# i3drobotics/i3dr_stereo_camera-ros

Hardware: AMD Instinct MI355X
Metric: stereo pairs/sec + ms/frame, 1920×1080 D=256 8-path SGM, 1/2/4/8 MI355X (higher is better)
Workload: dtype u8

## Files before the change

### i3dr_stereo_camera-ros_amd/csrc/census_sgm.hip

```cpp
#include "sgm_device.h"
#include "sgm_launch.h"

#include <atomic>
#include <string>

#ifndef SGM_WPE
#define SGM_WPE 4
#endif
#ifndef SGM_WPE32
#define SGM_WPE32 4
#endif
#ifndef SGM_NT_STORE
#define SGM_NT_STORE 1
#endif
#ifndef SGM_NT_LOAD
#define SGM_NT_LOAD 1
#endif
#ifndef SGM_EXP
#define SGM_EXP 0
#endif
#if SGM_EXP != 0 && !defined(SGM_EXPERIMENT_BUILD)
#error "SGM_EXP builds give invalid results: define SGM_EXPERIMENT_BUILD as well (never in a release build)"
#endif
#ifndef SGM_LRPRIO_HW
#define SGM_LRPRIO_HW 37
#endif
#ifndef SGM_LRPRIO_DIAG
#define SGM_LRPRIO_DIAG 64
#endif
#ifndef SGM_UPWTA_PRIO
#define SGM_UPWTA_PRIO 0
#endif
#ifndef SGM_ROWS_LPL8
#define SGM_ROWS_LPL8 0
#endif
#ifndef SGM_P32
#define SGM_P32 1
#endif

#include <algorithm>
#include <cstdio>
#include <cstdlib>
#include <vector>

namespace sgm {

#define SGM_CENSUS_BIT(B)                                                              \
    asm("v_cmp_lt_u32_sdwa vcc, %1, %2 src0_sel:BYTE_" #B " src1_sel:DWORD\n\t"      \
        "v_addc_co_u32_e32 %0, vcc, %0, %0, vcc"                                       \
        : "+v"(acc) : "v"(w), "v"(c) : "vcc")
__device__ __forceinline__ void census_bit(uint32_t& acc, uint32_t w, uint32_t c, int b)
{
    switch (b) {
    case 0: SGM_CENSUS_BIT(0); break;
    case 1: SGM_CENSUS_BIT(1); break;
    case 2: SGM_CENSUS_BIT(2); break;
    default: SGM_CENSUS_BIT(3); break;
    }
}
#undef SGM_CENSUS_BIT

template <int PITCH>
__device__ __forceinline__ uint64_t census_code_lds(const uint8_t* tile, int ty, int tx)
{
    static_assert(PITCH % 4 == 0, "u32 rows");
    const uint32_t* t32 = (const uint32_t*)tile + (PITCH / 4) * ty + (tx >> 2);
    const int sb = tx & 3;
    const uint32_t c = tile[(ty + 3) * PITCH + tx + 4];
    uint32_t lo = 0, hi = 0;
#pragma unroll
    for (int dy = 6; dy >= 0; dy--) {
        const uint32_t* r = t32 + (PITCH / 4) * dy;
        const uint32_t w0 = r[0], w1 = r[1], w2 = r[2];
        const uint32_t a0 = __builtin_amdgcn_alignbyte(w1, w0, sb);
        const uint32_t a1 = __builtin_amdgcn_alignbyte(w2, w1, sb);
        const uint32_t a2 = __builtin_amdgcn_alignbyte(w2, w2, sb);
#pragma unroll
        for (int dx = 8; dx >= 0; dx--) {
            if (dy == 3 && dx == 4) continue;
            const int k = dy * 9 + dx - (dy * 9 + dx > 31 ? 1 : 0);
            const uint32_t w = dx < 4 ? a0 : dx < 8 ? a1 : a2;
            if (k >= 32) census_bit(hi, w, c, dx & 3);
            else census_bit(lo, w, c, dx & 3);
        }
    }
    return (uint64_t)lo | ((uint64_t)hi << 32);
}

__global__ __launch_bounds__(256) void k_census9x7(const uint8_t* __restrict__ L, const uint8_t* __restrict__ R,
                                                   size_t stride, int W, int H,
                                                   uint64_t* __restrict__ cL, uint64_t* __restrict__ cR, int ch, int gray)
{
    __shared__ __attribute__((aligned(16))) uint8_t tile[10 * 72];
    const uint8_t* img = blockIdx.z ? R : L;
    uint64_t* out = blockIdx.z ? cR : cL;
    const int x0 = blockIdx.x * 64, y0 = blockIdx.y * 4;
    if (ch == 3) {
        for (int i = threadIdx.x; i < 10 * 72; i += 256) {
            int ty = i / 72, tx = i - ty * 72;
            int yy = min(max(y0 + ty - 3, 0), H - 1), xx = min(max(x0 + tx - 4, 0), W - 1);
            const uint8_t* s = img + (size_t)yy * stride + 3 * xx;
            tile[i] = (uint8_t)gray_px(s[0], s[1], s[2], gray);
        }
    } else {
        for (int i = threadIdx.x; i < 10 * 72; i += 256) {
            int ty = i / 72, tx = i - ty * 72;
            int yy = min(max(y0 + ty - 3, 0), H - 1), xx = min(max(x0 + tx - 4, 0), W - 1);
            tile[i] = img[(size_t)yy * stride + xx];
        }
    }
    __syncthreads();
    const int tx = threadIdx.x & 63, ty = threadIdx.x >> 6;
    const int x = x0 + tx, y = y0 + ty;
    if (x >= W || y >= H) return;
    out[(size_t)y * W + x] = census_code_lds<72>(tile, ty, tx);
}

template <int DPL>
__device__ __forceinline__ void wload(const uint8_t* src, uint32_t (&wd)[(DPL + 3) / 4])
{
    if constexpr (DPL == 2) { wd[0] = *(const uint16_t*)src; }
    else if constexpr (DPL == 4) { wd[0] = *(const uint32_t*)src; }
    else if constexpr (DPL == 8) { const uint2 v = *(const uint2*)src; wd[0] = v.x; wd[1] = v.y; }
    else {
#pragma unroll
        for (int q = 0; q < DPL / 16; q++) {
            const uint4 v = ((const uint4*)src)[q];
            wd[4 * q] = v.x; wd[4 * q + 1] = v.y; wd[4 * q + 2] = v.z; wd[4 * q + 3] = v.w;
        }
    }
}

template <int DPL>
__device__ __forceinline__ void wload_buf(const uint8_t* base, uint32_t off, uint32_t (&wd)[(DPL + 3) / 4])
{
    const __amdgpu_buffer_rsrc_t rs = __builtin_amdgcn_make_buffer_rsrc((void*)base, 0, 0x7FFFFFFF, 0x00020000);
    constexpr int aux = SGM_NT_LOAD ? 2 : 0;
    if constexpr (DPL == 2) { wd[0] = __builtin_amdgcn_raw_buffer_load_b16(rs, off, 0, aux); }
    else if constexpr (DPL == 4) { wd[0] = __builtin_amdgcn_raw_buffer_load_b32(rs, off, 0, aux); }
    else if constexpr (DPL == 8) {
        const auto v = __builtin_amdgcn_raw_buffer_load_b64(rs, off, 0, aux);
        wd[0] = v[0]; wd[1] = v[1];
    } else {
#pragma unroll
        for (int q = 0; q < DPL / 16; q++) {
            const auto v = __builtin_amdgcn_raw_buffer_load_b128(rs, off + 16 * q, 0, aux);
            wd[4 * q] = v[0]; wd[4 * q + 1] = v[1]; wd[4 * q + 2] = v[2]; wd[4 * q + 3] = v[3];
        }
    }
}

template <int DPL>
__device__ __forceinline__ void store_pairs(uint8_t* dst, uint8_t* dst_hi, const uint32_t (&L)[DPL / 2])
{
    if constexpr (DPL == 2) {
        const uint16_t v = (uint16_t)__builtin_amdgcn_perm(0u, L[0], 0x0c0c0200u);
        if constexpr (SGM_NT_STORE) __builtin_nontemporal_store(v, (uint16_t*)dst);
        else *(uint16_t*)dst = v;
    } else if constexpr (DPL == 4) {
        const uint32_t v = __builtin_amdgcn_perm(L[1], L[0], 0x06040200u);
        if constexpr (SGM_NT_STORE) __builtin_nontemporal_store(v, (uint32_t*)dst);
        else *(uint32_t*)dst = v;
    } else if constexpr (DPL == 8) {
        typedef unsigned int v2u __attribute__((ext_vector_type(2)));
        const v2u v = {__builtin_amdgcn_perm(L[1], L[0], 0x06040200u), __builtin_amdgcn_perm(L[3], L[2], 0x06040200u)};
        if constexpr (SGM_NT_STORE) __builtin_nontemporal_store(v, (v2u*)dst);
        else *(v2u*)dst = v;
    } else {
        typedef unsigned int v4u __attribute__((ext_vector_type(4)));
#pragma unroll
        for (int q = 0; q < DPL / 16; q++) {
            const v4u v = {__builtin_amdgcn_perm(L[8 * q + 1], L[8 * q + 0], 0x06040200u),
                           __builtin_amdgcn_perm(L[8 * q + 3], L[8 * q + 2], 0x06040200u),
                           __builtin_amdgcn_perm(L[8 * q + 5], L[8 * q + 4], 0x06040200u),
                           __builtin_amdgcn_perm(L[8 * q + 7], L[8 * q + 6], 0x06040200u)};
            v4u* d = (v4u*)(q == 0 ? dst : dst_hi);
            if constexpr (SGM_NT_STORE) __builtin_nontemporal_store(v, d);
            else *d = v;
        }
    }
}

constexpr uint32_t kBaseP = 0x6400u, kBaseP2 = 0x64006400u;
constexpr uint32_t kInfP = 0x7000u, kInfP2 = 0x70007000u;
// ... 117 lines not shown
    HChunk16 c;
    c.cl = cLr[min(max(x, 0), g.W - 1)];
    const int xr = DX > 0 ? x + 1 - g.minD : x - g.minD - LPL * DPL;
    c.inj = cRr[min(max(xr, 0), g.W - 1)];
    return c;
}

template <int DPL, bool EXACT, int DX, bool PRIO = false, int LPL = 16>
__device__ __forceinline__ void p16_horiz(const uint64_t* __restrict__ cL, const uint64_t* __restrict__ cR,
                                          uint8_t* __restrict__ V, uint8_t* __restrict__ trash, const Geom& g,
                                          int y0)
{
    static_assert(LPL == 16 || LPL == 32, "horizontal scans: 16- or 32-lane lines");
    constexpr int M = DPL / 2;
    constexpr int U = DPL > 16 ? DPL : 16;
    const int lane = threadIdx.x & 63;
    const int r = lane / LPL, p = lane % LPL;
    const int y = y0 + r;
    const bool rowok = y < g.H;
    const int yc = min(y, g.H - 1);
    const uint64_t* cLr = cL + (size_t)yc * g.W;
    const uint64_t* cRr = cR + (size_t)yc * g.W;
    uint32_t imask[M], start[M];
    make_imask<DPL, EXACT, LPL>(p, g.D, imask, start);
    const uint32_t P1P1 = (uint32_t)g.P1 * 0x10001u, P2P2 = ((uint32_t)g.P2 + kBaseP) * 0x10001u;
    const int n = g.width1;
    const int xfirst = DX > 0 ? g.minX1 : g.maxX1 - 1;
    uint64_t cr[DPL];
#pragma unroll
    for (int k = 0; k < DPL; k++) cr[k] = cRr[min(max(xfirst - g.minD - p * DPL - k, 0), g.W - 1)];
    uint32_t Lr[M];
#pragma unroll
    for (int i = 0; i < M; i++) Lr[i] = start[i];
    uint8_t* rowbase = V + (size_t)yc * g.width1 * g.D + p * DPL;
    uint8_t* tr = trash + lane * DPL;
    const bool lane_ok = rowok && (EXACT || p * DPL < g.D);
    const bool hi_ok = EXACT || p * DPL + 16 < g.D;
    HChunk16 cur = hload16<DPL, DX, LPL>(cLr, cRr, g, 0, lane & 15);
    HChunk16 nxt = cur;
    for (int b = 0; b * U < n; b++) {
        if constexpr (PRIO) lr_prio(((n - b * U) * SGM_LRPRIO_HW) >> 6, g.H);
        static_for<0, U>([&](auto tc) {
            constexpr int t = decltype(tc)::value;
            if constexpr (t % 16 == 0) nxt = hload16<DPL, DX, LPL>(cLr, cRr, g, (b * U + t) / 16 + 1, lane & 15);
            const int i = b * U + t;
            const uint64_t cl = row_bcast_u64<t % 16>(cur.cl);
            const uint64_t inj = row_bcast_u64<t % 16>(cur.inj);
            uint32_t Labs[M];
            p16_step<DPL, EXACT, LPL>(Lr, cl, [&](int k) { return cr[DX > 0 ? ((k - t) % DPL + DPL) % DPL : (k + t) % DPL]; },
                                      P1P1, P2P2, imask, Labs);
            const int x1 = DX > 0 ? i : n - 1 - i;
            const bool ok = lane_ok && i < n;
            uint8_t* dst = ok ? rowbase + (size_t)x1 * g.D : tr;
            store_pairs<DPL>(dst, (ok && hi_ok) ? dst + 16 : tr + 16, Labs);
            if constexpr (DX > 0) {
                constexpr int ph = ((DPL - 1 - t) % DPL + DPL) % DPL;
                cr[ph] = LPL == 32 ? line32_shr1_u64(cr[ph], inj) : row_shr1_u64(cr[ph], inj);
            } else {
                constexpr int ph = t % DPL;
                cr[ph] = LPL == 32 ? line32_shl1_u64(cr[ph], inj) : row_shl1_u64(cr[ph], inj);
            }
            if constexpr (t % 16 == 15) cur = nxt;
        });
    }
}

template <int DPL, int LPL>
struct RowSeg {
    static constexpr int NL = kWG / LPL;
    static constexpr int NSEG = LPL * DPL + NL - 1;
    static constexpr int NPAD = LPL >= 16 ? NSEG + NSEG / 16 + 1 : NSEG + 4 * (NSEG / 32) + 4;
    static constexpr int NTOT = NSEG + NL;
    static constexpr int NLOAD = (NTOT + kWG - 1) / kWG;
    static constexpr int BUF = NPAD + NL + kWG;
    static __device__ __forceinline__ int phys(int e) { return LPL >= 16 ? e + (e >> 4) : e + 4 * (e >> 5); }
};
template <int DPL16>
struct RowsCfg {
#if SGM_ROWS_LPL8
    static constexpr int LPL = DPL16 <= 16 ? 8 : LineCfg<DPL16>::LPL;
#else
    static constexpr int LPL = LineCfg<DPL16>::LPL;
#endif
    static constexpr int DPL = DPL16 * 16 / LPL;
    static constexpr int NL = kWG / LPL;
};

template <int DPL, int LPL>
using SegRegs = uint64_t[RowSeg<DPL, LPL>::NLOAD];
template <int DPL, int LPL>
struct SegAddr {
    uint32_t off[RowSeg<DPL, LPL>::NLOAD];
    const char* lo;
};
template <int DPL, int LPL>
__device__ __forceinline__ SegAddr<DPL, LPL> seg_addr(const uint64_t* cL, const uint64_t* cR, const Geom& g, int tid)
{
    using RS = RowSeg<DPL, LPL>;
    SegAddr<DPL, LPL> a;
    const uint64_t* base = cL < cR ? cL : cR;
    const int bias = LPL * DPL + max(g.minD, 0);
    a.lo = (const char*)base - (size_t)8 * bias;
#pragma unroll
    for (int m = 0; m < RS::NLOAD; m++) {
        const int q = min(tid + m * kWG, RS::NTOT - 1);
        const int rel = q < RS::NSEG ? (int)(cR - base) + q - g.minD - LPL * DPL + 1 : (int)(cL - base) + (q - RS::NSEG);
        a.off[m] = (uint32_t)(8 * (rel + bias));
    }
    return a;
}
template <int DPL, int LPL>
__device__ __forceinline__ void seg_load(SegRegs<DPL, LPL>& v, const SegAddr<DPL, LPL>& a,
                                         const Geom& g, int rx, int ry, int xb, int s)
{
    const int y = ry > 0 ? s : g.H - 1 - s;
    const int yc = (SGM_EXP & 1) ? 0 : min(max(y, 0), g.H - 1);
    const char* sb = a.lo + (size_t)8 * ((size_t)yc * g.W + (xb + rx * s));
#pragma unroll
    for (int m = 0; m < RowSeg<DPL, LPL>::NLOAD; m++) v[m] = *(const uint64_t*)(sb + a.off[m]);
}

template <int DPL, int LPL>
__device__ __forceinline__ void seg_store(uint64_t* buf, const SegRegs<DPL, LPL>& v, int tid)
{
    using RS = RowSeg<DPL, LPL>;
#pragma unroll
    for (int m = 0; m < RS::NLOAD; m++) {
        const int q0 = tid + m * kWG;
        const int at = q0 < RS::NSEG ? RS::phys(q0) : (q0 < RS::NTOT ? RS::NPAD + (q0 - RS::NSEG) : RS::NPAD + RS::NL + tid);
        buf[at] = v[m];
    }
}

template <int DPL, bool EXACT, int LPL>
__device__ __forceinline__ void p16_seed(const uint8_t* src, const uint32_t (&imask)[DPL / 2], uint32_t (&Lr)[DPL / 2])
{
    uint32_t wd[(DPL + 3) / 4], Labs[DPL / 2];
    wload<DPL>(src, wd);
#pragma unroll
    for (int i = 0; i < DPL / 2; i++) {
        const uint32_t pr = __builtin_amdgcn_perm(0u, wd[i / 2], (i & 1) ? 0x0c030c02u : 0x0c010c00u);
        Labs[i] = pr | kBaseP2;
        if (!EXACT) Labs[i] = pk_max(Labs[i], imask[i]);
    }
    p16_relative<DPL, LPL>(Labs, Lr);
}

struct UpWta {
    const uint8_t* vols;
    size_t vol_bytes;
    uint64_t* res;
};
struct WtaPix { int best, minS, d16; bool rej; };
template <int DPL, bool EXACT>
__device__ __forceinline__ WtaPix wta_pix16(const uint32_t (&E)[(DPL + 3) / 4], const uint32_t (&O)[(DPL + 3) / 4],
                                            int p, const Geom& g, float inv_u, uint32_t* srow);
template <int DPL, bool EXACT>
__device__ __forceinline__ void wta_emask(int p, const Geom& g, uint32_t (&emaskE)[(DPL + 3) / 4],
                                          uint32_t (&emaskO)[(DPL + 3) / 4]);
template <int DPL>
__host__ __device__ constexpr size_t upwta_lds_bytes() { return (size_t)8 * 2 * RowSeg<DPL, 16>::BUF + (size_t)16 * 32 * ((DPL + 3) / 4) * 4; }

template <int DPL, bool EXACT, int LPL, bool FUSE = false, bool PRIO = false, int NP = 8>
__device__ __forceinline__ void p16_rows(const uint64_t* __restrict__ cL, const uint64_t* __restrict__ cR,
                                         uint8_t* __restrict__ V, uint8_t* __restrict__ trash, const Geom& g, int dir,
                                         int xb, const PathLaunch16& pl, uint64_t* lds, const UpWta& uw = UpWta{})
{
    static_assert(!FUSE || LPL == 16, "up+WTA blocks use 16 lanes per line (the WTA layout)");
    using RS = RowSeg<DPL, LPL>;
    constexpr int M = DPL / 2;
    constexpr int NL = RS::NL;
    const int tid = threadIdx.x;
    const int lane = tid & 63, w = tid >> 6;
    const int r = lane >> 4;
    const int p = LPL == 32 ? lane & 31 : LPL == 16 ? lane & 15 : (lane & 15) >> 1;
    const int j = LPL == 32 ? 2 * w + (lane >> 5) : LPL == 16 ? 4 * w + r : 8 * w + 2 * r + (lane & 1);
    const int rx = dir_rx(dir), ry = dir_ry(dir);
    int s0, s1;
    if (rx == 0) { s0 = 0; s1 = g.H; }
    else if (rx > 0) { s0 = max(0, g.minX1 - xb - (NL - 1)); s1 = min(g.H, g.maxX1 - xb); }
    else { s0 = max(0, xb - g.maxX1 + 1); s1 = min(g.H, xb + NL - g.minX1); }
    if (s0 >= s1) return;
    uint32_t imask[M], start[M];
    make_imask<DPL, EXACT, LPL>(p, g.D, imask, start);
    const uint32_t P1P1 = (uint32_t)g.P1 * 0x10001u, P2P2 = ((uint32_t)g.P2 + kBaseP) * 0x10001u;
    uint32_t Lr[M];
#pragma unroll
    for (int i = 0; i < M; i++) Lr[i] = start[i];
    bool pv = false;
    const uint8_t* bnd = pl.bnd[ry > 0 ? 0 : 1];
    if (bnd && s0 == 0) {
        const int x = xb + j, xp = x - rx;
        const bool cont = x >= g.minX1 && x < g.maxX1 && xp >= g.minX1 && xp < g.maxX1;
        const int xs = min(max(xp, g.minX1), g.maxX1 - 1) - g.minX1;
        uint32_t Ls[M];
        p16_seed<DPL, EXACT, LPL>(bnd + bnd_slot_of(dir) * pl.bnd_slot + (size_t)xs * g.D + p * DPL, imask, Ls);
#pragma unroll
        for (int i = 0; i < M; i++) Lr[i] = cont ? Ls[i] : Lr[i];
        pv = cont;
    }
    const bool lane_act = EXACT || p * DPL < g.D;
    const bool hi_ok = EXACT || p * DPL + 16 < g.D;
    uint8_t* const tr = trash + (tid & 63) * DPL;
    const int e_hi = j + (LPL - p) * DPL - 1;

    uint64_t* buf0 = lds;
    uint64_t* buf1 = lds + RS::BUF;
    uint64_t R0[RS::NLOAD], R1[RS::NLOAD], R2[RS::NLOAD], R3[RS::NLOAD];
    const SegAddr<DPL, LPL> sa = seg_addr<DPL, LPL>(cL, cR, g, tid);
    seg_load<DPL, LPL>(R0, sa, g, rx, ry, xb, s0);
    seg_store<DPL, LPL>(buf0, R0, tid);
    seg_load<DPL, LPL>(R1, sa, g, rx, ry, xb, min(s0 + 1, s1 - 1));
    seg_load<DPL, LPL>(R2, sa, g, rx, ry, xb, min(s0 + 2, s1 - 1));
    seg_load<DPL, LPL>(R3, sa, g, rx, ry, xb, min(s0 + 3, s1 - 1));
    __syncthreads();

    constexpr int NWD = (DPL + 3) / 4;
    constexpr int NV = NP - 1;
    uint32_t vw[NV][NWD], emaskE[NWD], emaskO[NWD];
    uint32_t* srow = (uint32_t*)(lds + 2 * RS::BUF) + j * 32 * NWD;
    const float inv_u = 1.0f / (float)max(100 - g.uniq, 1);
    const uint32_t voff = (uint32_t)((min(max(xb + j, g.minX1), g.maxX1 - 1) - g.minX1) * g.D + (lane_act ? p * DPL : 0));
    uint64_t vols0 = (uint64_t)uw.vols;
    if constexpr (FUSE) asm volatile("" : "+s"(vols0));
    auto vload = [&](int s) {
        const uint8_t* rb = (const uint8_t*)vols0 + (size_t)max(g.H - 1 - s, 0) * g.width1 * g.D;
#pragma unroll
        for (int k = 0; k < NV; k++) wload_buf<DPL>(rb + (size_t)(k == 0 ? 0 : k + 1) * uw.vol_bytes, voff, vw[k]);
    };
    if constexpr (FUSE) {
        wta_emask<DPL, EXACT>(p, g, emaskE, emaskO);
        vload(s0);
    }
    const uint64_t* resrow = FUSE ? uw.res + (size_t)(g.H - 1 - s0) * g.W : nullptr;
    auto step = [&](int s, const uint64_t* bufc) {
        const int x = xb + j + rx * s;
        const bool valid = s < s1 && x >= g.minX1 && x < g.maxX1;
        const int y = ry > 0 ? s : g.H - 1 - s;
        const uint64_t cl = bufc[RS::NPAD + j];
        uint32_t Labs[M];
        uint32_t E[NWD], O[NWD];
        if constexpr (FUSE) {
#pragma unroll
            for (int jj = 0; jj < NWD; jj++) {
                uint32_t e = 0, o = 0;
#pragma unroll
                for (int k = 0; k < NV; k++) {
                    e += vw[k][jj] & 0x00FF00FFu;
                    o += __builtin_amdgcn_perm(0u, vw[k][jj], 0x0c030c01u);
                }
                asm("" : "+v"(e), "+v"(o));
                E[jj] = e;
                O[jj] = o;
            }
        }
        const uint32_t P2x = pv ? P2P2 : kBaseP2;
        if constexpr (FUSE) __builtin_amdgcn_sched_barrier(0);
        p16_step<DPL, EXACT, LPL>(Lr, cl, [&](int k) { return bufc[RS::phys(e_hi - k)]; }, P1P1, P2x, imask, Labs);
        if constexpr (FUSE) {
            __builtin_amdgcn_sched_barrier(0);
#pragma unroll
            for (int jj = 0; jj < NWD; jj++) {
                const uint32_t a = Labs[2 * jj], b = 2 * jj + 1 < M ? Labs[2 * jj + 1] : 0u;
                E[jj] = (E[jj] + __builtin_amdgcn_perm(b, a, 0x0c040c00u)) | emaskE[jj];
                O[jj] = (O[jj] + __builtin_amdgcn_perm(b, a, 0x0c060c02u)) | emaskO[jj];
            }
            vload(s + 1);
            __builtin_amdgcn_sched_barrier(0);
            const WtaPix px = wta_pix16<DPL, EXACT>(E, O, p, g, inv_u, srow);
            const uint64_t v = (uint64_t)(uint16_t)(px.rej ? g.invalid : px.d16) |
                               ((uint64_t)(uint16_t)(px.rej ? -1 : px.best) << 16) | ((uint64_t)(uint16_t)px.minS << 32);
            const __amdgpu_buffer_rsrc_t rr = __builtin_amdgcn_make_buffer_rsrc((void*)resrow, 0, g.W * 8, 0x00020000);
            resrow -= g.W;
            typedef unsigned int v2u __attribute__((ext_vector_type(2)));
            __builtin_amdgcn_raw_buffer_store_b64(__builtin_bit_cast(v2u, v), rr,
                                                  (valid && p == 0) ? (uint32_t)x * 8u : 0x80000000u, 0, 2);
        } else {
            const bool ok = valid && lane_act && !((SGM_EXP & 2) && dir == 1);
            uint8_t* const vrow = V + (size_t)min(max(y, 0), g.H - 1) * g.width1 * g.D;
            uint8_t* const dst = ok ? vrow + (uint32_t)((x - g.minX1) * g.D + p * DPL) : tr;
            store_pairs<DPL>(dst, (ok && hi_ok) ? dst + 16 : tr + 16, Labs);
        }
        pv = valid;
    };
    auto body = [&](int s, const uint64_t* bcur, uint64_t* bnext, uint64_t (&Rnext)[RS::NLOAD],
                    uint64_t (&Rfree)[RS::NLOAD]) {
        seg_load<DPL, LPL>(Rfree, sa, g, rx, ry, xb, min(s + 4, s1 - 1));
        step(s, bcur);
        seg_store<DPL, LPL>(bnext, Rnext, tid);
        __syncthreads();
    };
    for (int s = s0; s < s1; s += 4) {
        if constexpr (PRIO) lr_prio(rx != 0 ? ((s1 - s) * SGM_LRPRIO_DIAG) >> 6 : s1 - s, g.H);
        body(s, buf0, buf1, R1, R0);
        body(s + 1, buf1, buf0, R2, R1);
        body(s + 2, buf0, buf1, R3, R2);
        body(s + 3, buf1, buf0, R0, R3);
    }
}

template <int DPL>
__host__ __device__ constexpr int rows_lds_codes() { return 2 * RowSeg<RowsCfg<DPL>::DPL, RowsCfg<DPL>::LPL>::BUF; }

template <int DPL, bool EXACT, bool PRIO = false, int NP = 0>
__device__ __forceinline__ void paths_block16(const PathFrames& pf, size_t vol_bytes, size_t trash_off,
                                              const Geom& g, const PathLaunch16& pl, uint32_t it, uint64_t* lds)
{
    using RC = RowsCfg<DPL>;
    using HC = LineCfg<DPL>;
    const int dir = (int)(it >> 24);
    const int f = (int)((it >> 22) & 3u);
    const int lb = (int)(it & 0x3FFFFFu);
    if (f >= pf.n || ((pf.skip_dirs >> dir) & 1u)) return;
    const uint64_t* cL = pick4(pf.cL, f);
    const uint64_t* cR = pick4(pf.cR, f);
    uint8_t* V = pick4(pf.vols, f) + (size_t)vol_slot(NP ? NP : pf.np, dir) * vol_bytes;
    uint8_t* trash = V + trash_off;
    const int y0 = lb * HC::HROWS + (64 / HC::LPL) * (threadIdx.x >> 6);
    if (dir == 6) p16_horiz<HC::DPL, EXACT, 1, PRIO, HC::LPL>(cL, cR, V, trash, g, y0);
    else if (dir == 7) p16_horiz<HC::DPL, EXACT, -1, PRIO, HC::LPL>(cL, cR, V, trash, g, y0);
    else p16_rows<RC::DPL, EXACT, RC::LPL, false, PRIO>(cL, cR, V, trash, g, dir, pl.xb_lo[dir] + lb * RC::NL, pl, lds);
}

__device__ __forceinline__ void trace_record(uint64_t* trace, uint64_t tag, uint64_t t0)
{
    const uint64_t t1 = __builtin_amdgcn_s_memrealtime();
    const uint32_t hw = __builtin_amdgcn_s_getreg((4 << 0) | (0 << 6) | (31 << 11));
    const uint32_t xcc = __builtin_amdgcn_s_getreg((20 << 0) | (0 << 6) | (15 << 11));
    uint64_t* r = trace + ((size_t)blockIdx.x * 4 + (threadIdx.x >> 6)) * 4;
    r[0] = tag | ((uint64_t)blockIdx.x << 32); r[1] = ((uint64_t)xcc << 32) | hw; r[2] = t0; r[3] = t1;
}

template <int DPL, bool EXACT>
__global__ __launch_bounds__(kWG) __attribute__((amdgpu_waves_per_eu(DPL >= 32 && !SGM_P32 ? SGM_WPE32 : SGM_WPE)))
void k_census_paths16(PathFrames pf, size_t vol_bytes, size_t trash_off, Geom g, PathLaunch16 pl,
                      const uint32_t* __restrict__ items, uint64_t* __restrict__ trace)
{
    __shared__ uint64_t lds[rows_lds_codes<DPL>()];
    const uint64_t t0 = trace ? __builtin_amdgcn_s_memrealtime() : 0;
    paths_block16<DPL, EXACT, true>(pf, vol_bytes, trash_off, g, pl, items[blockIdx.x], lds);
    if (trace && (threadIdx.x & 63) == 0)
        trace_record(trace, items[blockIdx.x], t0);
}

template <int DPL>
__host__ __device__ constexpr size_t wta_key_bytes(int W)
{
    return (size_t)kWG * 8 * ((DPL + 3) / 4) > (size_t)4 * W ? (size_t)kWG * 8 * ((DPL + 3) / 4) : (size_t)4 * W;
}
template <int DPL>
__host__ __device__ constexpr size_t wta_lds_bytes(int W) { return wta_key_bytes<DPL>(W) + RowLds::rest_bytes(W); }

template <int DPL, bool EXACT>
__device__ __forceinline__ WtaPix wta_pix16(const uint32_t (&E)[(DPL + 3) / 4], const uint32_t (&O)[(DPL + 3) / 4],
                                            int p, const Geom& g, float inv_u, uint32_t* srow)
{
    constexpr int NWD = (DPL + 3) / 4;
    constexpr int KB = DPL > 16 ? 5 : 4;
    constexpr uint32_t KMASK = (1u << KB) - 1;
    constexpr int G = pair_group(DPL);
    auto kof = [](int b) { return (uint32_t)(b < DPL ? vol_byte_d(G, b) : b) & KMASK; };
    uint32_t km = 0xFFFFFFFFu;
#pragma unroll
    for (int j = 0; j < NWD; j++) {
        uint32_t ce = (kof(4 * j + 2) << 16) | kof(4 * j), co = (kof(4 * j + 3) << 16) | kof(4 * j + 1);
        uint32_t ke, ko;
        if constexpr (EXACT && DPL >= 4) {
            asm("" : "+s"(ce), "+s"(co));
            ke = (E[j] << KB) | ce; ko = (O[j] << KB) | co;
        }
        else { ke = pk_shl(E[j], KB) | ce; ko = pk_shl(O[j], KB) | co; }
        km = pk_min(km, pk_min(ke, ko));
    }
    km = pk_min(km, alignbit16(km, km)) & 0xFFFFu;
    const uint32_t kmin = row_min_u32(((km >> KB) << 9) | (uint32_t)(p * DPL + (int)(km & KMASK)));
    WtaPix r;
    const int best = (int)(kmin & 511u);
    const int minS = (int)(kmin >> 9);
#pragma unroll
    for (int j = 0; j < NWD; j++) { srow[p * 2 * NWD + j] = E[j]; srow[p * 2 * NWD + NWD + j] = O[j]; }
    auto s_at = [&](int d) {
        const int kk = vol_d_byte(G, d % DPL);
        const uint32_t v = srow[(d / DPL) * 2 * NWD + (kk & 1) * NWD + (kk >> 2)];
        return (int)((v >> (16 * ((kk >> 1) & 1))) & 0xFFFFu);
    };
    const int sm = s_at(max(best - 1, 0)), sp = s_at(min(best + 1, 16 * DPL - 1));
    int T = 0;
    if (g.uniq < 100) {
        if (minS > 0) {
            const int num = minS * 100 - 1, den = 100 - g.uniq;
            int q = (int)((float)num * inv_u);
            q += (q + 1) * den <= num ? 1 : 0;
            q -= q * den > num ? 1 : 0;
            T = min(q + 1, 8 * 255 + 1);
        }
    } else {
        T = (minS == 0 && g.uniq > 100) ? 1 : 0;
    }
    const uint32_t TT = (uint32_t)T * 0x10001u;
    uint32_t acc = 0;
#pragma unroll
    for (int j = 0; j < NWD; j++) acc += pk_subs(TT, E[j]) + pk_subs(TT, O[j]);
    const int tot = (int)row_sum_u32(__builtin_amdgcn_sad_u16(acc, 0u, 0u));
    const int win = max(T - minS, 0) + (best > 0 ? max(T - sm, 0) : 0) + (best < g.D - 1 ? max(T - sp, 0) : 0);
    int outside = tot - win;
    if (g.uniq >= 100) {
        const int nwin = 1 + (best > 0 ? 1 : 0) + (best < g.D - 1 ? 1 : 0);
        outside = minS > 0 ? g.D - nwin : (g.uniq > 100 ? (g.D - nwin) - outside : 0);
    }
    r.rej = outside > 0;
    const int den = max(sm + sp - 2 * minS, 1);
    const bool use = g.subpix && best > 0 && best < g.D - 1;
    r.d16 = best * 16 + (use ? tdiv_rcp((sm - sp) * 16 + den, 2 * den) : 0) + g.minD * 16;
    r.best = best;
    r.minS = minS;
    return r;
}

template <int DPL, bool EXACT>
__device__ __forceinline__ void wta_emask(int p, const Geom& g, uint32_t (&emaskE)[(DPL + 3) / 4],
                                          uint32_t (&emaskO)[(DPL + 3) / 4])
{
#pragma unroll
    for (int j = 0; j < (DPL + 3) / 4; j++) {
        auto bad = [&](int b) { return b >= DPL || (!EXACT && p * DPL + vol_byte_d(pair_group(DPL), b) >= g.D); };
        emaskE[j] = (bad(4 * j) ? 0xFFFFu : 0u) | (bad(4 * j + 2) ? 0xFFFF0000u : 0u);
        emaskO[j] = (bad(4 * j + 1) ? 0xFFFFu : 0u) | (bad(4 * j + 3) ? 0xFFFF0000u : 0u);
    }
}

template <int DPL, bool EXACT, int NP, typename OutT = int16_t>
__device__ __forceinline__ void wta_row16(const uint8_t* __restrict__ vols, size_t vol_bytes, const Geom& g,
                                          OutT* __restrict__ out, size_t out_stride, int y, uint32_t* lds)
{
    constexpr int NWD = (DPL + 3) / 4;
    uint32_t* sl = lds;
    RowLds R(lds, (char*)lds + wta_key_bytes<DPL>(g.W), g.W);
    const int tid = threadIdx.x, lane = tid & 63;
    const int w = __builtin_amdgcn_readfirstlane(tid >> 6);
    const int r = lane >> 4, p = lane & 15;
    R.init(g, tid, kWG, false);
    const bool lane_act = EXACT || p * DPL < g.D;
    const size_t row0 = (size_t)y * g.width1 * g.D;
    const uint32_t off0 = (uint32_t)(lane_act ? p * DPL : 0);
    uint32_t* srow = sl + (w * 4 + r) * 32 * NWD;
    uint32_t emaskE[NWD], emaskO[NWD];
    wta_emask<DPL, EXACT>(p, g, emaskE, emaskO);
    const float inv_u = 1.0f / (float)max(100 - g.uniq, 1);
    const int n = g.width1;
    const int nq = (n + 3) / 4;
    const uint32_t loff = off0 + (uint32_t)(r * g.D);
    auto load = [&](int q, uint32_t (&v)[NP][NWD]) {
        const uint8_t* rowq = vols + row0 + (size_t)(4 * q) * g.D;
#pragma unroll
        for (int vv = 0; vv < NP; vv++) {
            if ((SGM_EXP & 4) && vv == 1) { for (int j = 0; j < NWD; j++) v[vv][j] = 0; continue; }
            wload_buf<DPL>(rowq + (size_t)vv * vol_bytes, loff, v[vv]);
        }
    };
    uint32_t E[NWD], O[NWD];
    auto sum8 = [&](const uint32_t (&v)[NP][NWD]) {
#pragma unroll
        for (int j = 0; j < NWD; j++) {
            uint32_t e = 0, o = 0;
#pragma unroll
            for (int vv = 0; vv < NP; vv++) {
                e += v[vv][j] & 0x00FF00FFu;
                o += __builtin_amdgcn_perm(0u, v[vv][j], 0x0c030c01u);
            }
            E[j] = e | emaskE[j];
            O[j] = o | emaskO[j];
        }
    };
    uint32_t nxt[NP][NWD];
    load(min(w, nq - 1), nxt);
    sum8(nxt);
    for (int q = w; q < nq; q += 4) {
        load(min(q + 4, nq - 1), nxt);
        const WtaPix px = wta_pix16<DPL, EXACT>(E, O, p, g, inv_u, srow);
        const int x1 = 4 * q + r;
        const bool wr = p == 0 && x1 < n;
        const int x = wr ? g.minX1 + x1 : g.W + lane;
        R.bst[x] = (int16_t)(px.rej ? -1 : px.best);
        R.mins[x] = (uint16_t)px.minS;
        R.drow[(wr && !px.rej) ? x : g.W + lane] = (int16_t)px.d16;
        sum8(nxt);
    }
    R.init_key(g, tid, kWG);
    row_finish(g, tid, kWG, R.drow, R.bst, R.mins, R.key, (int16_t*)R.mins, out + (size_t)y * out_stride);
}

template <int DPL, bool EXACT, int NP>
__device__ __forceinline__ void wta_block16(const WtaFrames& wf, size_t vol_bytes, const Geom& g, size_t out_stride,
                                            int b, uint32_t* lds)
{
    const int f = b / g.H;
    wta_row16<DPL, EXACT, NP>(pick4(wf.vols, f), vol_bytes, g, pick4(wf.out, f), out_stride, b - f * g.H, lds);
}

template <int DPL, bool EXACT, int NP>
__global__ __launch_bounds__(kWG) void k_census_wta16(WtaFrames wf, size_t vol_bytes, Geom g, size_t out_stride)
{
    extern __shared__ uint32_t lds_dyn[];
    wta_block16<DPL, EXACT, NP>(wf, vol_bytes, g, out_stride, blockIdx.x, lds_dyn);
}

template <int DPL, bool EXACT, int NP>
__global__ __launch_bounds__(kWG) void k_census_wta16f(WtaFrames wf, size_t vol_bytes, Geom g)
{
    extern __shared__ uint32_t lds_dyn[];
    wta_row16<DPL, EXACT, NP, float>(wf.vols[0], vol_bytes, g, wf.outf[0], wf.outf_stride, blockIdx.x, lds_dyn);
}

constexpr int kCensusRows = 32;

__device__ __forceinline__ void census_block(const CensusFrames& cf, int W, int H, int b, uint8_t* tile)
{
    const int bx = (W + 63) / 64, per_img = bx * ((H + kCensusRows - 1) / kCensusRows);
    const int img = b / per_img, r = b - img * per_img;
    const int f = img >> 1, by = r / bx;
    const uint8_t* src = (img & 1) ? pick4(cf.R, f) : pick4(cf.L, f);
    uint64_t* out = (img & 1) ? pick4(cf.cR, f) : pick4(cf.cL, f);
    const int x0 = (r - by * bx) * 64, y0 = by * kCensusRows;
    constexpr int TH = kCensusRows + 6;
    if (cf.ch == 3) {
        if (cf.rect.tab) {
            const float* mx = (img & 1) ? cf.rect.map[2] : cf.rect.map[0];
            const float* my = (img & 1) ? cf.rect.map[3] : cf.rect.map[1];
            uint8_t* rect = (img & 1) ? pick4(cf.rectR, f) : pick4(cf.rectL, f);
            for (int i = threadIdx.x; i < TH * 72; i += kWG) {
                const int ty = i / 72, tx = i - ty * 72;
                const int yy = min(max(y0 + ty - 3, 0), H - 1), xx = min(max(x0 + tx - 4, 0), W - 1);
                const size_t m = (size_t)yy * cf.rect.map_stride + xx;
                const uint32_t v = remap_cubic_px3(src, cf.stride, cf.rect.src_w, cf.rect.src_h, mx[m], my[m], cf.rect.tab);
                tile[i] = (uint8_t)gray_px(v & 255, (v >> 8) & 255, v >> 16, cf.gray);
                if (rect && ty >= 3 && ty < 3 + kCensusRows && tx >= 4 && tx < 68 && y0 + ty - 3 < H && x0 + tx - 4 < W) {
                    uint8_t* d = rect + (size_t)yy * cf.rect_stride + 3 * xx;
                    d[0] = (uint8_t)v;
                    d[1] = (uint8_t)(v >> 8);
                    d[2] = (uint8_t)(v >> 16);
                }
            }
        } else {
            for (int i = threadIdx.x; i < TH * 72; i += kWG) {
                const int ty = i / 72, tx = i - ty * 72;
                const int yy = min(max(y0 + ty - 3, 0), H - 1), xx = min(max(x0 + tx - 4, 0), W - 1);
                const uint8_t* s = src + (size_t)yy * cf.stride + 3 * xx;
                tile[i] = (uint8_t)gray_px(s[0], s[1], s[2], cf.gray);
            }
        }
    } else if (cf.rect.tab) {
        const float* mx = (img & 1) ? cf.rect.map[2] : cf.rect.map[0];
        const float* my = (img & 1) ? cf.rect.map[3] : cf.rect.map[1];
        uint8_t* rect = (img & 1) ? pick4(cf.rectR, f) : pick4(cf.rectL, f);
        for (int i = threadIdx.x; i < TH * 72; i += kWG) {
            const int ty = i / 72, tx = i - ty * 72;
            const int yy = min(max(y0 + ty - 3, 0), H - 1), xx = min(max(x0 + tx - 4, 0), W - 1);
            const size_t m = (size_t)yy * cf.rect.map_stride + xx;
            const uint8_t v = remap_cubic_px(src, cf.stride, cf.rect.src_w, cf.rect.src_h, mx[m], my[m], cf.rect.tab);
            tile[i] = v;
            if (rect && ty >= 3 && ty < 3 + kCensusRows && tx >= 4 && tx < 68 && y0 + ty - 3 < H && x0 + tx - 4 < W)
                rect[(size_t)yy * cf.rect_stride + xx] = v;
        }
    } else {
        for (int i = threadIdx.x; i < TH * 72; i += kWG) {
            const int ty = i / 72, tx = i - ty * 72;
            const int yy = min(max(y0 + ty - 3, 0), H - 1), xx = min(max(x0 + tx - 4, 0), W - 1);
            tile[i] = src[(size_t)yy * cf.stride + xx];
        }
    }
    __syncthreads();
    const int tx = threadIdx.x & 63, x = x0 + tx;
    if (x >= W) return;
    for (int ty = threadIdx.x >> 6; ty < kCensusRows; ty += kWG / 64) {
        const int y = y0 + ty;
        if (y >= H) break;
        out[(size_t)y * W + x] = census_code_lds<72>(tile, ty, tx);
    }
}

__global__ __launch_bounds__(kWG) void k_census_tiles(CensusFrames cf, int W, int H)
{
    __shared__ __attribute__((aligned(16))) uint8_t tile[(kCensusRows + 6) * 72];
    census_block(cf, W, H, blockIdx.x, tile);
}

template <int DPL, bool EXACT, int NP>
__global__ __launch_bounds__(kWG) __attribute__((amdgpu_waves_per_eu(DPL >= 32 ? SGM_WPE32 : SGM_WPE)))
void k_census_fused16(PathFrames pf, WtaFrames wf, CensusFrames cf, size_t vol_bytes, size_t trash_off, Geom g,
                      PathLaunch16 pl, const uint32_t* __restrict__ items, int n_items, size_t out_stride,
                      int period16, int wta_rows, uint64_t* __restrict__ trace)
{
    extern __shared__ uint64_t lds_dyn64[];
    const uint64_t t0 = trace ? __builtin_amdgcn_s_memrealtime() : 0;
    const int b = blockIdx.x;
    const int n_wta = wta_rows ? g.H * wf.n : 0;
    auto wcount = [&](int bb) {
        int w = period16 > 0 ? min((bb + 1) * 16 / period16, n_wta) : 0;
        return max(w, bb + 1 - n_items);
    };
    int kind = 2, idx = b - n_items - n_wta;
    if (b < n_items + n_wta) {
        const int w = wcount(b);
        const bool is_wta = w > (b > 0 ? wcount(b - 1) : 0);
        kind = is_wta ? 1 : 0;
        idx = is_wta ? w - 1 : b - w;
    }
    if (kind == 0) {
        const uint32_t it = items[idx];
        if constexpr (DPL > 16) {
            paths_block16<DPL, EXACT, false, NP>(pf, vol_bytes, trash_off, g, pl, it, lds_dyn64);
        } else if ((it >> 24) == 8u) {
            const int f = (int)((it >> 22) & 3u);
            if (f < wf.n) {
#if SGM_UPWTA_PRIO
                __builtin_amdgcn_s_setprio(SGM_UPWTA_PRIO);
#endif
                const UpWta uw{pick4(wf.vols, f), vol_bytes, pick4(wf.res, f)};
                p16_rows<DPL, EXACT, 16, true, false, NP>(pick4(wf.cL, f), pick4(wf.cR, f), nullptr, nullptr, g, 1,
                                               pl.xb_lo[1] + (int)(it & 0x3FFFFFu) * 16, pl, lds_dyn64, uw);
            }
        } else {
            paths_block16<DPL, EXACT, false, NP>(pf, vol_bytes, trash_off, g, pl, it, lds_dyn64);
        }
    } else if (kind == 1) {
        wta_block16<DPL, EXACT, NP>(wf, vol_bytes, g, out_stride, idx, (uint32_t*)lds_dyn64);
    } else {
        census_block(cf, g.W, g.H, idx, (uint8_t*)lds_dyn64);
    }
    if (trace && (threadIdx.x & 63) == 0)
        trace_record(trace, (kind == 0 ? items[idx] : 0u) | ((uint64_t)kind << 62), t0);
}
// ... 219 lines not shown
```

Baseline: 749.5.

## Defer fused up+WTA tail to batched flush, add LDS threshold table, cheaper byte sums

In the fused up-path + WTA kernel, per-step results (best, minS, neighbours, threshold, total) are packed into LDS, and the uniqueness tail plus result store run once every 16 steps across lanes. Before, all 16 lanes of a line computed the tail and only lane 0 stored. A per-block LDS table of uniqueness thresholds replaces the per-pixel float-divide threshold computation when DPL is at least 16. The even/odd byte summation drops one AND per volume by subtracting the shifted odd sum. This costs extra LDS, a table-fill pass before the first barrier, and more complex store addressing.

```diff
diff --git a/i3dr_stereo_camera-ros_amd/csrc/census_sgm.hip b/i3dr_stereo_camera-ros_amd/csrc/census_sgm.hip
--- a/i3dr_stereo_camera-ros_amd/csrc/census_sgm.hip
+++ b/i3dr_stereo_camera-ros_amd/csrc/census_sgm.hip
@@ -30,6 +30,9 @@
 #endif
 #ifndef SGM_UPWTA_PRIO
 #define SGM_UPWTA_PRIO 0
+#endif
+#ifndef SGM_UPWTA_TTAB
+#define SGM_UPWTA_TTAB 16
 #endif
 #ifndef SGM_ROWS_LPL8
 #define SGM_ROWS_LPL8 0
@@ -453,14 +456,43 @@
     uint64_t* res;
 };
 struct WtaPix { int best, minS, d16; bool rej; };
-template <int DPL, bool EXACT>
+template <int NV, int NWD>
+__device__ __forceinline__ void sum_eo(const uint32_t (&v)[NV][NWD], int j, uint32_t& e, uint32_t& o)
+{
+    static_assert(NV * 255 < 65536, "the even halves must not carry");
+    uint32_t sv = 0, so = 0;
+#pragma unroll
+    for (int k = 0; k < NV; k++) {
+        sv += v[k][j];
+        so += __builtin_amdgcn_perm(0u, v[k][j], 0x0c030c01u);
+    }
+    e = sv - (so << 8);
+    o = so;
+}
+struct WtaTot { int best, minS, sm, sp, T, tot; };
+template <int DPL, bool EXACT, typename TF>
+__device__ __forceinline__ WtaTot wta_tot16(const uint32_t (&E)[(DPL + 3) / 4], const uint32_t (&O)[(DPL + 3) / 4],
+                                            int p, TF thresh, uint32_t* srow);
+__device__ __forceinline__ WtaPix wta_tail(const WtaTot& t, const Geom& g);
+template <int DPL, bool EXACT, typename TF>
 __device__ __forceinline__ WtaPix wta_pix16(const uint32_t (&E)[(DPL + 3) / 4], const uint32_t (&O)[(DPL + 3) / 4],
-                                            int p, const Geom& g, float inv_u, uint32_t* srow);
+                                            int p, const Geom& g, TF thresh, uint32_t* srow)
+{
+    return wta_tail(wta_tot16<DPL, EXACT>(E, O, p, thresh, srow), g);
+}
+__device__ __forceinline__ int wta_thresh(int minS, int uniq, float inv_u);
 template <int DPL, bool EXACT>
 __device__ __forceinline__ void wta_emask(int p, const Geom& g, uint32_t (&emaskE)[(DPL + 3) / 4],
                                           uint32_t (&emaskO)[(DPL + 3) / 4]);
+constexpr int kThreshN = 2048;
+__host__ __device__ constexpr bool upwta_ttab(int dpl) { return dpl >= SGM_UPWTA_TTAB; }
+__host__ __device__ constexpr int upwta_line_dwords(int nwd) { return 32 * nwd + 17 * 4; }
 template <int DPL>
-__host__ __device__ constexpr size_t upwta_lds_bytes() { return (size_t)8 * 2 * RowSeg<DPL, 16>::BUF + (size_t)16 * 32 * ((DPL + 3) / 4) * 4; }
+__host__ __device__ constexpr size_t upwta_lds_bytes()
+{
+    return (size_t)8 * 2 * RowSeg<DPL, 16>::BUF + (size_t)16 * upwta_line_dwords((DPL + 3) / 4) * 4 +
+           (upwta_ttab(DPL) ? (size_t)kThreshN * 2 : 0);
+}
 
 template <int DPL, bool EXACT, int LPL, bool FUSE = false, bool PRIO = false, int NP = 8>
 __device__ __forceinline__ void p16_rows(const uint64_t* __restrict__ cL, const uint64_t* __restrict__ cR,
@@ -514,13 +546,17 @@
     seg_load<DPL, LPL>(R1, sa, g, rx, ry, xb, min(s0 + 1, s1 - 1));
     seg_load<DPL, LPL>(R2, sa, g, rx, ry, xb, min(s0 + 2, s1 - 1));
     seg_load<DPL, LPL>(R3, sa, g, rx, ry, xb, min(s0 + 3, s1 - 1));
+    constexpr int NWD = (DPL + 3) / 4;
+    const uint16_t* ttab = (const uint16_t*)((uint32_t*)(lds + 2 * RS::BUF) + 16 * upwta_line_dwords(NWD));
+    const float inv_u = 1.0f / (float)max(100 - g.uniq, 1);
+    if constexpr (FUSE && upwta_ttab(DPL)) {
+        for (int i = tid; i < kThreshN; i += kWG) ((uint16_t*)ttab)[i] = (uint16_t)wta_thresh(i, g.uniq, inv_u);
+    }
     __syncthreads();
 
-    constexpr int NWD = (DPL + 3) / 4;
     constexpr int NV = NP - 1;
     uint32_t vw[NV][NWD], emaskE[NWD], emaskO[NWD];
-    uint32_t* srow = (uint32_t*)(lds + 2 * RS::BUF) + j * 32 * NWD;
-    const float inv_u = 1.0f / (float)max(100 - g.uniq, 1);
+    uint32_t* srow = (uint32_t*)(lds + 2 * RS::BUF) + j * upwta_line_dwords(NWD);
     const uint32_t voff = (uint32_t)((min(max(xb + j, g.minX1), g.maxX1 - 1) - g.minX1) * g.D + (lane_act ? p * DPL : 0));
     uint64_t vols0 = (uint64_t)uw.vols;
     if constexpr (FUSE) asm volatile("" : "+s"(vols0));
@@ -533,8 +569,27 @@
         wta_emask<DPL, EXACT>(p, g, emaskE, emaskO);
         vload(s0);
     }
-    const uint64_t* resrow = FUSE ? uw.res + (size_t)(g.H - 1 - s0) * g.W : nullptr;
-    auto step = [&](int s, const uint64_t* bufc) {
+    typedef unsigned int v4u __attribute__((ext_vector_type(4)));
+    v4u* const keep = (v4u*)(srow + 32 * NWD);
+    auto flush = [&](int sb) {
+        int pp = p, xl = xb + j;
+        asm volatile("" : "+v"(pp), "+v"(xl));
+        const v4u k = keep[pp];
+        const WtaTot t{(int)(k.x & 511u), (int)(k.x >> 9), (int)(k.y & 0xFFFFu), (int)(k.y >> 16), (int)k.z, (int)k.w};
+        const WtaPix px = wta_tail(t, g);
+        const uint64_t v = (uint64_t)(uint16_t)(px.rej ? g.invalid : px.d16) |
+                           ((uint64_t)(uint16_t)(px.rej ? -1 : px.best) << 16) | ((uint64_t)(uint16_t)px.minS << 32);
+        const int s = sb + pp;
+        const int x = xl + rx * s;
+        const int ytop = g.H - 1 - sb, ylo = max(ytop - 15, 0);
+        const bool ok = s < s1 && x >= g.minX1 && x < g.maxX1;
+        const __amdgpu_buffer_rsrc_t rr = __builtin_amdgcn_make_buffer_rsrc((void*)(uw.res + (size_t)ylo * g.W), 0,
+                                                                            (ytop - ylo + 1) * g.W * 8, 0x00020000);
+        typedef unsigned int v2u __attribute__((ext_vector_type(2)));
+        __builtin_amdgcn_raw_buffer_store_b64(__builtin_bit_cast(v2u, v), rr,
+                                              ok ? (uint32_t)((ytop - pp - ylo) * g.W + x) * 8u : 0x80000000u, 0, 2);
+    };
+    auto step = [&](int s, const uint64_t* bufc, bool first) {
         const int x = xb + j + rx * s;
         const bool valid = s < s1 && x >= g.minX1 && x < g.maxX1;
         const int y = ry > 0 ? s : g.H - 1 - s;
@@ -544,16 +599,13 @@
         if constexpr (FUSE) {
 #pragma unroll
             for (int jj = 0; jj < NWD; jj++) {
-                uint32_t e = 0, o = 0;
-#pragma unroll
-                for (int k = 0; k < NV; k++) {
-                    e += vw[k][jj] & 0x00FF00FFu;
-                    o += __builtin_amdgcn_perm(0u, vw[k][jj], 0x0c030c01u);
-                }
+                uint32_t e, o;
+                sum_eo<NV, NWD>(vw, jj, e, o);
                 asm("" : "+v"(e), "+v"(o));
                 E[jj] = e;
                 O[jj] = o;
             }
+            if (first && s != s0 && ((s - s0) & 15) == 0) flush(s - 16);
         }
         const uint32_t P2x = pv ? P2P2 : kBaseP2;
         if constexpr (FUSE) __builtin_amdgcn_sched_barrier(0);
@@ -568,14 +620,10 @@
             }
             vload(s + 1);
             __builtin_amdgcn_sched_barrier(0);
-            const WtaPix px = wta_pix16<DPL, EXACT>(E, O, p, g, inv_u, srow);
-            const uint64_t v = (uint64_t)(uint16_t)(px.rej ? g.invalid : px.d16) |
-                               ((uint64_t)(uint16_t)(px.rej ? -1 : px.best) << 16) | ((uint64_t)(uint16_t)px.minS << 32);
-            const __amdgpu_buffer_rsrc_t rr = __builtin_amdgcn_make_buffer_rsrc((void*)resrow, 0, g.W * 8, 0x00020000);
-            resrow -= g.W;
-            typedef unsigned int v2u __attribute__((ext_vector_type(2)));
-            __builtin_amdgcn_raw_buffer_store_b64(__builtin_bit_cast(v2u, v), rr,
-                                                  (valid && p == 0) ? (uint32_t)x * 8u : 0x80000000u, 0, 2);
+            const WtaTot t = wta_tot16<DPL, EXACT>(E, O, p, [&](int minS) {
+                return upwta_ttab(DPL) ? (int)ttab[minS] : wta_thresh(minS, g.uniq, inv_u); }, srow);
+            keep[(s - s0) & 15] = (v4u){(uint32_t)t.best | ((uint32_t)t.minS << 9), (uint32_t)t.sm | ((uint32_t)t.sp << 16),
+                                        (uint32_t)t.T, (uint32_t)t.tot};
         } else {
             const bool ok = valid && lane_act && !((SGM_EXP & 2) && dir == 1);
             uint8_t* const vrow = V + (size_t)min(max(y, 0), g.H - 1) * g.width1 * g.D;
@@ -585,19 +633,20 @@
         pv = valid;
     };
     auto body = [&](int s, const uint64_t* bcur, uint64_t* bnext, uint64_t (&Rnext)[RS::NLOAD],
-                    uint64_t (&Rfree)[RS::NLOAD]) {
+                    uint64_t (&Rfree)[RS::NLOAD], bool first = false) {
         seg_load<DPL, LPL>(Rfree, sa, g, rx, ry, xb, min(s + 4, s1 - 1));
-        step(s, bcur);
+        step(s, bcur, first);
         seg_store<DPL, LPL>(bnext, Rnext, tid);
         __syncthreads();
     };
     for (int s = s0; s < s1; s += 4) {
         if constexpr (PRIO) lr_prio(rx != 0 ? ((s1 - s) * SGM_LRPRIO_DIAG) >> 6 : s1 - s, g.H);
-        body(s, buf0, buf1, R1, R0);
+        body(s, buf0, buf1, R1, R0, true);
         body(s + 1, buf1, buf0, R2, R1);
         body(s + 2, buf0, buf1, R3, R2);
         body(s + 3, buf1, buf0, R0, R3);
     }
+    if constexpr (FUSE) flush(s0 + ((s1 - s0 - 1) & ~15));
 }
 
 template <int DPL>
@@ -652,9 +701,9 @@
 template <int DPL>
 __host__ __device__ constexpr size_t wta_lds_bytes(int W) { return wta_key_bytes<DPL>(W) + RowLds::rest_bytes(W); }
 
-template <int DPL, bool EXACT>
-__device__ __forceinline__ WtaPix wta_pix16(const uint32_t (&E)[(DPL + 3) / 4], const uint32_t (&O)[(DPL + 3) / 4],
-                                            int p, const Geom& g, float inv_u, uint32_t* srow)
+template <int DPL, bool EXACT, typename TF>
+__device__ __forceinline__ WtaTot wta_tot16(const uint32_t (&E)[(DPL + 3) / 4], const uint32_t (&O)[(DPL + 3) / 4],
+                                            int p, TF thresh, uint32_t* srow)
 {
     constexpr int NWD = (DPL + 3) / 4;
     constexpr int KB = DPL > 16 ? 5 : 4;
@@ -675,7 +724,6 @@
     }
     km = pk_min(km, alignbit16(km, km)) & 0xFFFFu;
     const uint32_t kmin = row_min_u32(((km >> KB) << 9) | (uint32_t)(p * DPL + (int)(km & KMASK)));
-    WtaPix r;
     const int best = (int)(kmin & 511u);
     const int minS = (int)(kmin >> 9);
 #pragma unroll
@@ -686,23 +734,36 @@
         return (int)((v >> (16 * ((kk >> 1) & 1))) & 0xFFFFu);
     };
     const int sm = s_at(max(best - 1, 0)), sp = s_at(min(best + 1, 16 * DPL - 1));
+    const int T = thresh(minS);
+    const uint32_t TT = (uint32_t)T * 0x10001u;
+    uint32_t acc = 0;
+#pragma unroll
+    for (int j = 0; j < NWD; j++) acc += pk_subs(TT, E[j]) + pk_subs(TT, O[j]);
+    const int tot = (int)row_sum_u32(__builtin_amdgcn_sad_u16(acc, 0u, 0u));
+    return WtaTot{best, minS, sm, sp, T, tot};
+}
+
+__device__ __forceinline__ int wta_thresh(int minS, int uniq, float inv_u)
+{
     int T = 0;
-    if (g.uniq < 100) {
+    if (uniq < 100) {
         if (minS > 0) {
-            const int num = minS * 100 - 1, den = 100 - g.uniq;
+            const int num = minS * 100 - 1, den = 100 - uniq;
             int q = (int)((float)num * inv_u);
             q += (q + 1) * den <= num ? 1 : 0;
             q -= q * den > num ? 1 : 0;
             T = min(q + 1, 8 * 255 + 1);
         }
     } else {
-        T = (minS == 0 && g.uniq > 100) ? 1 : 0;
-    }
-    const uint32_t TT = (uint32_t)T * 0x10001u;
-    uint32_t acc = 0;
-#pragma unroll
-    for (int j = 0; j < NWD; j++) acc += pk_subs(TT, E[j]) + pk_subs(TT, O[j]);
-    const int tot = (int)row_sum_u32(__builtin_amdgcn_sad_u16(acc, 0u, 0u));
+        T = (minS == 0 && uniq > 100) ? 1 : 0;
+    }
+    return T;
+}
+
+__device__ __forceinline__ WtaPix wta_tail(const WtaTot& t, const Geom& g)
+{
+    const int best = t.best, minS = t.minS, sm = t.sm, sp = t.sp, T = t.T, tot = t.tot;
+    WtaPix r;
     const int win = max(T - minS, 0) + (best > 0 ? max(T - sm, 0) : 0) + (best < g.D - 1 ? max(T - sp, 0) : 0);
     int outside = tot - win;
     if (g.uniq >= 100) {
@@ -763,12 +824,8 @@
     auto sum8 = [&](const uint32_t (&v)[NP][NWD]) {
 #pragma unroll
         for (int j = 0; j < NWD; j++) {
-            uint32_t e = 0, o = 0;
-#pragma unroll
-            for (int vv = 0; vv < NP; vv++) {
-                e += v[vv][j] & 0x00FF00FFu;
-                o += __builtin_amdgcn_perm(0u, v[vv][j], 0x0c030c01u);
-            }
+            uint32_t e, o;
+            sum_eo<NP, NWD>(v, j, e, o);
             E[j] = e | emaskE[j];
             O[j] = o | emaskO[j];
         }
@@ -778,7 +835,7 @@
     sum8(nxt);
     for (int q = w; q < nq; q += 4) {
         load(min(q + 4, nq - 1), nxt);
-        const WtaPix px = wta_pix16<DPL, EXACT>(E, O, p, g, inv_u, srow);
+        const WtaPix px = wta_pix16<DPL, EXACT>(E, O, p, g, [&](int minS) { return wta_thresh(minS, g.uniq, inv_u); }, srow);
         const int x1 = 4 * q + r;
         const bool wr = p == 0 && x1 < n;
         const int x = wr ? g.minX1 + x1 : g.W + lane;
```

After: 764.6 (median of 6 runs). 1.02x the previous value.
